# Ham3798/shielded-pool-pinocchio-solana

Hardware: AMD Instinct MI355X
Metric: Groth16 proofs/sec (higher is better)
Workload: dtype u32x8 (254-bit Montgomery integers); 1 GPU; audit_circuit (RLWE, const-PK; scripts/generate_audit.py:246-465), batch of 2048 independent proofs per GPU per step, every row a distinct witness; circuit=audit, n_constraints=29178, n_wires=35432, domain=32768, batch_per_gpu=2048, n_distinct_witnesses=2048, table_bytes=226725433344, parallelism=independent proofs x1, pk_bytes=9850060

## Files before the change

include/spp.h:

```cpp
#ifndef SPP_H
#define SPP_H
#include <stddef.h>
#include <stdint.h>
#ifdef __cplusplus
extern "C" {
#endif

#define SPP_OK 0
#define SPP_ERR_BAD_INPUT (-1)
#define SPP_ERR_NO_DEVICE (-2)
#define SPP_ERR_IO (-3)
#define SPP_ERR_UNSAT (-4)
#define SPP_ERR_HIP (-5)
#define SPP_ERR_NOT_IMPLEMENTED (-6)
#define SPP_ERR_FORMAT (-7)

#define SPP_CIRCUIT_WITHDRAW 1
#define SPP_CIRCUIT_AUDIT 2
#define SPP_CIRCUIT_WITHDRAW_REFSHAPE 3
#define SPP_CIRCUIT_WITHDRAW_DEPTH20 4

#define SPP_PROOF_LEN 388
#define SPP_WITHDRAW_PW_LEN 172
#define SPP_AUDIT_PW_LEN 76
// ... 142 lines not shown
int  spp_pool_submit_audit_batch(spp_pool*, size_t count, const uint8_t* proofs, const uint8_t* pws, int32_t* result);
int  spp_pool_withdraw_batch(spp_pool*, size_t count, const uint8_t* proofs, const uint8_t* pws, const uint8_t* recipients,
                             int32_t* result, uint64_t* amounts);
#define SPP_INSTR_DEPOSIT 0
#define SPP_INSTR_SUBMIT_AUDIT 1
#define SPP_INSTR_WITHDRAW 2
int  spp_pool_settle_log(spp_pool*, size_t count, const uint8_t* kinds,
                         size_t n_deposits, const uint8_t* roots,
                         size_t n_audits, const uint8_t* audit_proofs, const uint8_t* audit_pws,
                         size_t n_withdraws, const uint8_t* withdraw_proofs, const uint8_t* withdraw_pws, const uint8_t* recipients,
                         int32_t* result, uint64_t* amounts);

int spp_ntt_fr(spp_ctx* ctx, uint8_t* data, uint32_t logn, int inverse);
int spp_msm_g1(spp_ctx* ctx, const uint8_t* bases, const uint8_t* scalars, size_t n, int window_bits, uint8_t out[64]);
int spp_msm_g2(spp_ctx* ctx, const uint8_t* bases, const uint8_t* scalars, size_t n, int window_bits, uint8_t out[128]);

int spp_msm_g1_pippenger(spp_ctx* ctx, const uint8_t* bases, const uint8_t* scalars, size_t n, uint8_t out[64]);
int spp_msm_g2_pippenger(spp_ctx* ctx, const uint8_t* bases, const uint8_t* scalars, size_t n, uint8_t out[128]);
int spp_msm_g1_pippenger_bench(spp_ctx* ctx, size_t n, uint64_t seed, const uint8_t scale_be[32], int iters, uint8_t out[64],
                               float* ms_total, float* ms_bucket_kernel);
int spp_msm_g1_pippenger_bench_dist(spp_ctx* ctx, size_t n, uint64_t seed, uint32_t small_permille, const uint8_t scale_be[32], int iters,
                                    uint8_t out[64], float* ms_total, float* ms_bucket_kernel);
int spp_msm_g1_pippenger_bench_shard(spp_ctx* ctx, size_t n_total, size_t first, size_t count, uint64_t seed, uint32_t small_permille,
                                     const uint8_t scale_be[32], int iters, uint8_t out[64], float* ms_total, float* ms_bucket_kernel);

#ifdef __cplusplus
}
#endif
#endif
```

shielded-pool-pinocchio-solana_amd/csrc/f29.hpp:

```cpp
#pragma once
#include "bn254.hpp"

#if defined(__HIPCC__)
#define SPP_HD_COLD __host__ __device__ __attribute__((noinline))
#else
#define SPP_HD_COLD __attribute__((noinline))
#endif

namespace spp {

template <class Pm>
struct F29 {
  uint32_t l[9];
  using Base = Fp<Pm>;
  typedef uint32_t (*ConstFn)(int);
  static constexpr uint32_t M = (1u << 29) - 1u;
  static constexpr uint32_t INV = Pm::INV32 & M;
  static SPP_HD constexpr uint32_t P9(int k) { return Base::P9(k); }

  template <ConstFn C>
  static SPP_HD F29 konst() {
    F29 r;
    SPP_UNROLL for (int i = 0; i < 9; i++) r.l[i] = C(i);
    return r;
// ... 176 lines not shown
  }
  SPP_HD XYZZ<B> to_xyzz() const {
    if (inf) return XYZZ<B>::infinity();
    return {X.to_fp(), Y.to_fp(), ZZ.scaled_to_fp(), ZZZ.scaled_to_fp()};
  }
  static SPP_HD XYZZ29 from_xyzz(const XYZZ<B>& q) {
    XYZZ29 r;
    r.inf = q.is_inf();
    r.X = F::from_fp(q.X);
    r.Y = F::from_fp(q.Y);
    r.ZZ = F::from_fp(q.ZZ) * F::template konst<Pm::K29_IN>();
    r.ZZZ = F::from_fp(q.ZZZ) * F::template konst<Pm::K29_IN>();
    return r;
  }

  SPP_HD void madd(const Affine<B>& e, bool negate) {
    F x2 = F::from_words(e.x.l);
    F y2 = F::from_words(e.y.l);
    if (negate) y2 = F::template neg_lazy<Pm::SUBC_4P_1>(y2);
    if (inf) {
      X = x2 * F::template konst<Pm::K29_IN>();
      Y = y2 * F::template konst<Pm::K29_IN>();
      ZZ = F::template konst<Pm::K29_IN>();
      ZZZ = ZZ;
      inf = false;
      return;
    }
    const F U2 = x2 * ZZ;
    const F Pp = F::template sub_norm<Pm::SUBC_6P_1>(U2, X);
    if (Pp.template is_zero_mod_p<7>()) {
      const F S2 = y2 * ZZZ;
      const F Rr = F::template sub_norm<Pm::SUBC_2P_1>(S2, Y);
      if (Rr.template is_zero_mod_p<3>()) {
        XYZZ<B> t = to_xyzz();
        t.dbl_inplace();
        const XYZZ29 d = from_xyzz(t);
        X = d.X;
        Y = d.Y;
        ZZ = d.ZZ;
        ZZZ = d.ZZZ;
      } else {
        inf = true;
      }
      return;
    }
    const F PP = Pp.sqr();
    const F Q = X * PP;
    const F PPP = Pp * PP;
    ZZ = ZZ * PP;
    const F S2 = y2 * ZZZ;
    const F Rr = F::template sub_norm<Pm::SUBC_2P_1>(S2, Y);
    ZZZ = ZZZ * PPP;
    const F R2 = Rr.sqr();
    X = F::template sub3_norm<Pm::SUBC_4P_3>(R2, PPP, Q);
    const F T = F::template sub_lazy<Pm::SUBC_6P_1>(Q, X);
    const F Yn = F::template neg_lazy<Pm::SUBC_2P_1>(Y);
    Y = F::mul2(Rr, T, Yn, PPP);
  }
};

struct F29x2 {
  using F = F29<FqParams>;
  using Pm = FqParams;
  F c0, c1;

  static SPP_HD F29x2 from_words(const Fq2& a) { return {F::from_words(a.c0.l), F::from_words(a.c1.l)}; }
  template <F::ConstFn CA>
  static SPP_HD F29x2 mul(const F29x2& a, const F29x2& b) {
    const F na1 = F::template neg_lazy<CA>(a.c1);
    return {F::mul2(a.c0, b.c0, na1, b.c1), F::mul2(a.c0, b.c1, a.c1, b.c0)};
  }
  SPP_HD F29x2 mul_real(const F& k) const { return {c0 * k, c1 * k}; }
// ... 44 lines not shown
  SPP_HD XYZZ<Fq2> to_xyzz() const {
    if (inf) return XYZZ<Fq2>::infinity();
    return {X.to_fp(), Y.to_fp(), ZZ.scaled_to_fp(), ZZZ.scaled_to_fp()};
  }
  static SPP_HD XYZZ29G2 from_xyzz(const XYZZ<Fq2>& q) {
    XYZZ29G2 r;
    r.inf = q.is_inf();
    const F k = F::template konst<Pm::K29_IN>();
    r.X = E::from_fp(q.X);
    r.Y = E::from_fp(q.Y);
    r.ZZ = E::from_fp(q.ZZ).mul_real(k);
    r.ZZZ = E::from_fp(q.ZZZ).mul_real(k);
    return r;
  }

  SPP_HD void madd(const Affine<Fq2>& e, bool negate) {
    const E x2 = E::from_words(e.x);
    const E y2 = E::from_words(e.y);
    if (inf) {
      const F k = F::template konst<Pm::K29_IN>();
      X = x2.mul_real(k);
      const E yn = E::template neg_lazy<Pm::SUBC_4P_1>(y2);
      E ys;
      SPP_UNROLL for (int i = 0; i < 9; i++) {
        ys.c0.l[i] = negate ? yn.c0.l[i] : y2.c0.l[i];
        ys.c1.l[i] = negate ? yn.c1.l[i] : y2.c1.l[i];
      }
      Y = ys.mul_real(k);
      SPP_UNROLL for (int i = 0; i < 9; i++) {
        ZZ.c0.l[i] = k.l[i];
        ZZ.c1.l[i] = 0;
      }
      ZZZ = ZZ;
      inf = false;
      return;
    }
    const E U2 = E::template mul<Pm::SUBC_4P_1>(x2, ZZ);
    const E Pp = E::template sub_norm<Pm::SUBC_6P_1>(U2, X);
    E S2 = E::template mul<Pm::SUBC_4P_1>(y2, ZZZ);
    if (negate) S2 = E::template neg_lazy<Pm::SUBC_2P_1>(S2);
    const E Rr = E::template sub_norm<Pm::SUBC_2P_1>(S2, Y);
    if (Pp.template is_zero_mod_p<7>()) {
      if (Rr.template is_zero_mod_p<4>()) {
        XYZZ<Fq2> t = to_xyzz();
        t.dbl_inplace();
        const XYZZ29G2 d = from_xyzz(t);
        X = d.X;
        Y = d.Y;
        ZZ = d.ZZ;
        ZZZ = d.ZZZ;
      } else {
        inf = true;
      }
      return;
    }
    const E PP = Pp.template sqr<Pm::SUBC_8P_1>();
    const E Q = E::template mul<Pm::SUBC_6P_1>(X, PP);
    const E PPP = E::template mul<Pm::SUBC_8P_1>(Pp, PP);
    ZZ = E::template mul<Pm::SUBC_2P_1>(ZZ, PP);
    ZZZ = E::template mul<Pm::SUBC_2P_1>(ZZZ, PPP);
    const E R2 = Rr.template sqr<Pm::SUBC_6P_1>();
    X = E::template sub3_norm<Pm::SUBC_4P_3>(R2, PPP, Q);
    const E T = E::template sub_norm<Pm::SUBC_6P_1>(Q, X);
    const F nR1 = F::template neg_lazy<Pm::SUBC_6P_1>(Rr.c1);
    const F nY0 = F::template neg_lazy<Pm::SUBC_2P_1>(Y.c0);
    const F nY1 = F::template neg_lazy<Pm::SUBC_2P_1>(Y.c1);
    uint64_t c[18];
    F::clear(c);
    F::mac(c, Rr.c0, T.c0);
    F::mac(c, nR1, T.c1);
    F::mac(c, nY0, PPP.c0);
    F::mac(c, Y.c1, PPP.c1);
    const F y0 = F::reduce(c);
    F::clear(c);
    F::mac(c, Rr.c0, T.c1);
    F::mac(c, Rr.c1, T.c0);
    F::mac(c, nY0, PPP.c1);
    F::mac(c, nY1, PPP.c0);
    Y.c0 = y0;
    Y.c1 = F::reduce(c);
  }
};

}
```

shielded-pool-pinocchio-solana_amd/csrc/kernels.hpp:

```cpp
#pragma once
#include <hip/hip_runtime.h>
#include <stdint.h>
#include "bn254.hpp"
#include "msm_plan.hpp"
#include "msm_ragged.hpp"
#include "rlwe_ntt.hpp"

namespace spp {

struct DevSparse {
  const uint32_t* rowptr;
  const uint32_t* wire;
  const uint32_t* coeff;
  const uint32_t* lit;
};
static constexpr uint32_t COEFF_ONE = 0x80000000u;
static constexpr uint32_t COEFF_MINUS_ONE = 0x40000000u;
static constexpr uint32_t COEFF_MASK = 0x3fffffffu;

struct DevCircuit {
  DevSparse A, B, C, H;
  const Fr* coeffs;
  const Fr* aux;
  const uint32_t* program;
// ... 124 lines not shown
void launch_pool_commit(hipStream_t st, const PoolSet& set, uint64_t salt, const uint8_t* keys, uint32_t stride, uint32_t count, const int32_t* result,
                        uint32_t* set_count);
void launch_spmv_check(hipStream_t st, DevCircuit dc, const Fr* W, Fr* abc, uint32_t n, uint32_t P, uint32_t* status, int16_t* small = nullptr);

void launch_ntt(hipStream_t st, Fr* data, uint32_t logn, uint32_t P, const Fr* tw, bool dif, uint32_t nbatch, size_t batch_stride,
                const Fr* post = nullptr);
void launch_scale_rows(hipStream_t st, Fr* data, const Fr* table, uint32_t n, uint32_t P, uint32_t nbatch, size_t batch_stride);
void launch_qap_pointwise(hipStream_t st, Fr* abc, uint32_t n, uint32_t P, Fr zinv);
void launch_qap_product(hipStream_t st, Fr* abc, uint32_t n, uint32_t P);

template <class F>
struct MsmWalk;
template <>
struct MsmWalk<Fq> {
  static constexpr uint32_t waves_per_simd = 2;
  static constexpr bool gather_ahead = false;
};
template <>
struct MsmWalk<Fq2> {
  static constexpr uint32_t waves_per_simd = 1;
  static constexpr bool gather_ahead = true;
};
template <class F>
void launch_build_table(hipStream_t st, const Affine<F>* bases, uint32_t N, uint32_t c, uint32_t Wt, uint32_t row0, uint32_t nrows,
                        Affine<F>* table, XYZZ<F>* tmp, F* tmp_pre, const MsmBlock* blocks = nullptr, uint32_t E = 0);
void launch_msm_digits(hipStream_t st, const uint32_t* rows, const Fr* scalars, int16_t* dig, uint32_t N, uint32_t P, uint32_t c);
template <class F>
void launch_msm_accumulate(hipStream_t st, const Affine<F>* table, const MsmBlock* blocks, const int16_t* dig, XYZZ<F>* partial, uint32_t N, uint32_t P,
                           uint32_t c, const MsmPlan& pl, hipEvent_t ev_start = nullptr, hipEvent_t ev_stop = nullptr);
template <class F>
void launch_msm_reduce(hipStream_t st, XYZZ<F>* partial, XYZZ<F>* out, uint32_t P, const MsmPlan& pl, uint32_t c, bool empty);
static constexpr uint32_t MSM_FOLD_SETS = 8;
static constexpr uint32_t MSM_FOLD_RADIX = 8;
template <class F>
struct MsmFoldSets {
  XYZZ<F>* partial[MSM_FOLD_SETS];
  XYZZ<F>* out[MSM_FOLD_SETS];
  uint32_t Sg[MSM_FOLD_SETS], R[MSM_FOLD_SETS], c[MSM_FOLD_SETS];
  uint32_t cur[MSM_FOLD_SETS], half[MSM_FOLD_SETS];
};
template <class F>
void launch_msm_reduce_multi(hipStream_t st, MsmFoldSets<F> fs, uint32_t nsets, uint32_t P);

void launch_g1_eval_basis(hipStream_t st, const G1Affine* pts, uint32_t n_pts, uint32_t logn, const Fr* scale, const Fr* tw_inv, G1XYZZ* work,
// ... 34 lines not shown
```

shielded-pool-pinocchio-solana_amd/csrc/kernels_msm.hip:

```cpp
#include "msm_table.hpp"

namespace spp {

template void launch_build_table<Fq>(hipStream_t, const Affine<Fq>*, uint32_t, uint32_t, uint32_t, uint32_t, uint32_t, Affine<Fq>*,
                                     XYZZ<Fq>*, Fq*, const MsmBlock*, uint32_t);
template void launch_msm_accumulate<Fq>(hipStream_t, const Affine<Fq>*, const MsmBlock*, const int16_t*, XYZZ<Fq>*, uint32_t, uint32_t, uint32_t,
                                        const MsmPlan&, hipEvent_t, hipEvent_t);
template void launch_msm_reduce_multi<Fq>(hipStream_t, MsmFoldSets<Fq>, uint32_t, uint32_t);
template void launch_msm_reduce<Fq>(hipStream_t, XYZZ<Fq>*, XYZZ<Fq>*, uint32_t, const MsmPlan&, uint32_t, bool);
template void launch_fixed_base_mul<Fq>(hipStream_t, const Affine<Fq>*, uint32_t, const Fr*, uint32_t, Affine<Fq>*);

__global__ void __launch_bounds__(256) k_msm_digits(const uint32_t* __restrict__ rows, const Fr* __restrict__ scalars,
                                                    int16_t* __restrict__ dig, uint32_t N, uint32_t P, uint32_t Pp, uint32_t c, uint32_t W) {
  const uint64_t g = (uint64_t)blockIdx.x * blockDim.x + threadIdx.x;
  const uint32_t p = (uint32_t)(g % Pp), i = (uint32_t)(g / Pp);
  if (i >= N || p >= P) return;
  const Fr s = scalars[(size_t)rows[i] * P + p];
  uint32_t l[8];
  s.to_canonical(l);
  const bool neg = canonical_gt_half<FrParams>(l);
  if (neg) {
    uint32_t t[8];
    canonical_negate<FrParams>(l, t);
    SPP_UNROLL for (int k = 0; k < 8; k++) l[k] = t[k];
// ... 96 lines not shown
```

shielded-pool-pinocchio-solana_amd/csrc/kernels_msm_g2.hip:

```cpp
#include "msm_table.hpp"

namespace spp {

template void launch_build_table<Fq2>(hipStream_t, const Affine<Fq2>*, uint32_t, uint32_t, uint32_t, uint32_t, uint32_t, Affine<Fq2>*,
                                     XYZZ<Fq2>*, Fq2*, const MsmBlock*, uint32_t);
template void launch_msm_accumulate<Fq2>(hipStream_t, const Affine<Fq2>*, const MsmBlock*, const int16_t*, XYZZ<Fq2>*, uint32_t, uint32_t, uint32_t,
                                        const MsmPlan&, hipEvent_t, hipEvent_t);
template void launch_msm_reduce_multi<Fq2>(hipStream_t, MsmFoldSets<Fq2>, uint32_t, uint32_t);
template void launch_msm_reduce<Fq2>(hipStream_t, XYZZ<Fq2>*, XYZZ<Fq2>*, uint32_t, const MsmPlan&, uint32_t, bool);
template void launch_fixed_base_mul<Fq2>(hipStream_t, const Affine<Fq2>*, uint32_t, const Fr*, uint32_t, Affine<Fq2>*);

}
```

shielded-pool-pinocchio-solana_amd/csrc/msm_table.hpp:

```cpp
#pragma once
#include <hip/hip_ext.h>
#include "kernels.hpp"
#include <algorithm>
#include "f29.hpp"

namespace spp {

static constexpr unsigned MSM_FOLD_COOP_MAX_BATCH = 8;
static constexpr unsigned MSM_WALK_BLOCK = 64;

template <class F>
__global__ void __launch_bounds__(64) k_build_table(const Affine<F>* __restrict__ bases, uint32_t N, uint32_t E, uint32_t Wn,
                                                    uint32_t step_bits, uint32_t row0, uint32_t nrows, Affine<F>* __restrict__ table,
                                                    XYZZ<F>* __restrict__ tmp, F* __restrict__ tmp_pre, const MsmBlock* __restrict__ blocks) {
  const uint32_t rl = blockIdx.x * blockDim.x + threadIdx.x;
  if (rl >= nrows) return;
  const uint32_t row = row0 + rl;
  const size_t off = blocks ? (size_t)blocks[row >> 6].off : (size_t)(row >> 6) * E;
  Affine<F>* out = table + off * 64 + (row & 63);
  XYZZ<F>* t = tmp + rl;
  F* pre = tmp_pre + rl;
  if (row >= N * Wn) {
    for (uint32_t d = 0; d < E; d++) out[(size_t)d * 64] = Affine<F>::infinity();
    return;
// ... 71 lines not shown
__device__ __forceinline__ bool words_all_zero(const Fq& v) {
  uint32_t o = 0;
  SPP_UNROLL for (int i = 0; i < 8; i++) o |= v.l[i];
  return o == 0;
}
template <class F>
struct MsmAcc;
template <>
struct MsmAcc<Fq> {
  XYZZ29<FqParams> a;
  __device__ __forceinline__ void init() { a = XYZZ29<FqParams>::infinity(); }
  __device__ __forceinline__ void madd(const Affine<Fq>& e, bool sgn) {
    if (words_all_zero(e.x) && words_all_zero(e.y)) return;
    a.madd(e, sgn);
  }
  __device__ __forceinline__ XYZZ<Fq> result() const { return a.to_xyzz(); }
};

template <>
struct MsmAcc<Fq2> {
  XYZZ29G2 a;
  __device__ __forceinline__ void init() { a = XYZZ29G2::infinity(); }
  __device__ __forceinline__ void madd(const Affine<Fq2>& e, bool sgn) {
    if (words_all_zero(e.x.c0) && words_all_zero(e.x.c1) && words_all_zero(e.y.c0) && words_all_zero(e.y.c1)) return;
    a.madd(e, sgn);
  }
  __device__ __forceinline__ XYZZ<Fq2> result() const { return a.to_xyzz(); }
};


template <class F>
__global__ void __launch_bounds__(MSM_WALK_BLOCK, MsmWalk<F>::waves_per_simd) k_msm_flat(const Affine<F>* __restrict__ table, const MsmBlock* __restrict__ blocks,
                                                  const int16_t* __restrict__ dig, XYZZ<F>* __restrict__ partial, uint32_t N, uint32_t P,
                                                  uint32_t Pp, uint32_t R, uint32_t Sg) {
  const uint32_t g = blockIdx.x * blockDim.x + threadIdx.x;
  const uint32_t p = g % Pp, t = g / Pp;
  if (t >= R * Sg || p >= P) return;
  const uint32_t rho = t / Sg, sl = t % Sg;
  const int16_t* __restrict__ dg = dig + ((size_t)rho * N) * Pp + p;
  MsmAcc<F> acc;
  acc.init();
  if constexpr (MsmWalk<F>::gather_ahead) {
    int d_next = 0;
    Affine<F> e_next;
    for (uint32_t i0 = sl;; i0 += 4 * Sg) {
      const bool last = i0 >= N;
      uint64_t pack = 0;
      if (!last) {
        SPP_UNROLL for (uint32_t k = 0; k < 4; k++) {
          const uint32_t i = i0 + k * Sg;
          const uint32_t d = i < N ? (uint32_t)(uint16_t)dg[(size_t)i * Pp] : 0u;
          pack |= (uint64_t)d << (16 * k);
        }
      }
#pragma unroll 1
      for (uint32_t k = 0; k < 4; k++) {
        int d = (int)(int16_t)(uint16_t)(pack >> (16 * k));
        const bool flush = last && k == 0;
        const uint32_t i = i0 + k * Sg;
        const uint32_t mag = (uint32_t)(d < 0 ? -d : d);
        MsmBlock blk{};
        if (d != 0) blk = blocks[i >> 6];
        if (mag > blk.E) d = 0;
        if (d != 0 || flush) {
          Affine<F> e;
          if (d != 0) e = table[((size_t)blk.off + (mag - 1)) * 64 + (i & 63)];
          if (d_next != 0) acc.madd(e_next, d_next < 0);
          d_next = d;
          if (d != 0) e_next = e;
        }
      }
      if (last) break;
    }
  } else {
    for (uint32_t i0 = sl; i0 < N; i0 += 4 * Sg) {
      uint64_t pack = 0;
      SPP_UNROLL for (uint32_t k = 0; k < 4; k++) {
        const uint32_t i = i0 + k * Sg;
        const uint32_t d = i < N ? (uint32_t)(uint16_t)dg[(size_t)i * Pp] : 0u;
        pack |= (uint64_t)d << (16 * k);
      }
      if (pack == 0) continue;
#pragma unroll 1
      for (uint32_t k = 0; k < 4; k++) {
        const int d = (int)(int16_t)(uint16_t)(pack >> (16 * k));
        if (d != 0) {
          const uint32_t i = i0 + k * Sg;
          const uint32_t mag = (uint32_t)(d < 0 ? -d : d);
          const MsmBlock blk = blocks[i >> 6];
          if (mag <= blk.E) acc.madd(table[((size_t)blk.off + (mag - 1)) * 64 + (i & 63)], d < 0);
        }
      }
    }
  }
  partial[(size_t)t * P + p] = acc.result();
}

template <class F>
__global__ void __launch_bounds__(256) k_msm_rows(const Affine<F>* __restrict__ table, const int16_t* __restrict__ dig,
                                                  XYZZ<F>* __restrict__ partial, uint32_t N, uint32_t P, uint32_t Pp, uint32_t c,
                                                  uint32_t Wt, uint32_t R, uint32_t W, uint32_t Sg, uint32_t Q, uint32_t Wq) {
  const uint32_t g = blockIdx.x * blockDim.x + threadIdx.x;
  const uint32_t p = g % Pp, t = g / Pp;
  if (t >= R * Sg || p >= P) return;
  const uint32_t rho = t / Sg, sl = t % Sg;
  const uint32_t E = 1u << (c - 1);
  const size_t plane = (size_t)N * Pp;
  MsmAcc<F> acc;
  acc.init();
  const uint32_t items = N * Q;
// ... 10 lines not shown
      const uint32_t j = rho + R * m;
      if (j >= W) break;
      const int d = dg[(size_t)j * plane];
      if (d != 0) {
        const uint32_t row = i * Wt + m;
        const uint32_t mag = (uint32_t)(d < 0 ? -d : d);
        acc.madd(table[((size_t)(row >> 6) * E + (mag - 1)) * 64 + (row & 63)], d < 0);
      }
    }
  }
  partial[(size_t)t * P + p] = acc.result();
}

template <class F>
void launch_msm_accumulate(hipStream_t st, const Affine<F>* table, const MsmBlock* blocks, const int16_t* dig, XYZZ<F>* partial, uint32_t N, uint32_t P,
                           uint32_t c, const MsmPlan& pl, hipEvent_t ev_start, hipEvent_t ev_stop) {
  if (N == 0 || P == 0) {
    if (ev_start) hipEventRecord(ev_start, st);
    if (ev_stop) hipEventRecord(ev_stop, st);
    return;
  }
  const uint64_t lanes = (uint64_t)pl.R * pl.Sg * pl.Pp;
  if (pl.Wt == 1)
    hipExtLaunchKernelGGL(k_msm_flat<F>, dim3((uint32_t)((lanes + MSM_WALK_BLOCK - 1) / MSM_WALK_BLOCK)), dim3(MSM_WALK_BLOCK), 0, st, ev_start, ev_stop, 0, table, blocks, dig, partial, N, P, pl.Pp, pl.R, pl.Sg);
  else
    hipExtLaunchKernelGGL(k_msm_rows<F>, dim3((uint32_t)((lanes + 255) / 256)), dim3(256), 0, st, ev_start, ev_stop, 0, table, dig, partial, N, P, pl.Pp, c,
                          pl.Wt, pl.R, pl.W, pl.Sg, pl.Q, pl.Wq);
}

template <class T>
__device__ __forceinline__ T msm_shfl_xor(const T& v, int mask) {
  static_assert(sizeof(T) % 4 == 0, "word-sized");
  T r;
  const uint32_t* s = reinterpret_cast<const uint32_t*>(&v);
  uint32_t* d = reinterpret_cast<uint32_t*>(&r);
  SPP_UNROLL for (uint32_t i = 0; i < sizeof(T) / 4; i++) d[i] = (uint32_t)__shfl_xor((int)s[i], mask, 64);
  return r;
}
template <class F>
__global__ void __launch_bounds__(64) k_msm_fold_multi(MsmFoldSets<F> fs, uint32_t P, uint32_t coop) {
// ... 158 lines not shown
```

shielded-pool-pinocchio-solana_amd/csrc/spp_load.cpp:

```cpp
#include "spp_circuit.hpp"

static std::vector<PendingTable<Fq>>& pending(spp_circuit* c, Fq*) { return c->pending1; }
static std::vector<PendingTable<Fq2>>& pending(spp_circuit* c, Fq2*) { return c->pending2; }

static int upload_sparse(spp_circuit* c, const Circuit& circ, const Sparse& m, DevSparse* out) {
  std::vector<uint32_t> wire(m.terms.size()), coeff(m.terms.size()), lit(m.terms.size(), 0);
  Fr one = Fr::one(), mone = Fr::one().neg();
  std::vector<uint32_t> small(circ.coeffs.size(), 0);
  for (size_t ci = 0; ci < circ.coeffs.size(); ci++) {
    uint32_t v[8], nv[8];
    circ.coeffs[ci].to_canonical(v);
    bool hi0 = true;
    for (int k = 1; k < 8; k++) hi0 = hi0 && v[k] == 0;
    if (hi0 && v[0] != 0 && v[0] < (1u << 28)) { small[ci] = v[0]; continue; }
    circ.coeffs[ci].neg().to_canonical(nv);
    hi0 = true;
    for (int k = 1; k < 8; k++) hi0 = hi0 && nv[k] == 0;
    if (hi0 && nv[0] != 0 && nv[0] < (1u << 28)) small[ci] = nv[0] | 0x80000000u;
  }
  for (size_t i = 0; i < m.terms.size(); i++) {
    wire[i] = m.terms[i].wire;
    uint32_t ci = m.terms[i].coeff;
    uint32_t flag = 0;
    if (circ.coeffs[ci] == one) flag = COEFF_ONE;
// ... 798 lines not shown
  std::vector<uint32_t> rows(n);
  for (size_t i = 0; i < n; i++) {
    pts[i] = point_from_raw<F>(bases + PT_BYTES * i);
    sc[i] = Fr::from_bytes_be(scalars + 32 * i);
    rows[i] = (uint32_t)i;
  }
  spp_circuit tmpc;
  tmpc.ctx = ctx;
  tmpc.c_bits = cb;
  Affine<F>* table = nullptr;
  int e = build_table_chunked<F>(&tmpc, pts, cb, Wn, &table);
  Fr* d_sc = nullptr;
  uint32_t* d_rows = nullptr;
  XYZZ<F> *partial = nullptr, *d_out = nullptr;
  DevBuf dig;
  const MsmPlan pl = msm_plan((uint32_t)n, 1, cb, Wn, MsmWalk<F>::waves_per_simd, read_switches().msm);
  if (!e) e = own_upload(&tmpc, &d_sc, sc);
  if (!e) e = own_upload(&tmpc, &d_rows, rows);
  if (!e && hipMalloc((void**)&partial, sizeof(XYZZ<F>) * std::max<size_t>(pl.partial_elems(1), 1)) != hipSuccess) e = fail(SPP_ERR_HIP, "hipMalloc");
  if (!e && hipMalloc((void**)&d_out, sizeof(XYZZ<F>)) != hipSuccess) e = fail(SPP_ERR_HIP, "hipMalloc");
  if (!e && dig.alloc(sizeof(int16_t) * std::max<size_t>(msm_digit_elems((uint32_t)n, 1, cb), 1)) != hipSuccess) e = fail(SPP_ERR_HIP, "hipMalloc");
  XYZZ<F> res = XYZZ<F>::infinity();
  if (!e) {
    launch_msm_digits(st, d_rows, d_sc, dig.as<int16_t>(), (uint32_t)n, 1, cb);
    launch_msm_accumulate<F>(st, table, nullptr, dig.as<int16_t>(), partial, (uint32_t)n, 1, cb, pl);
    launch_msm_reduce<F>(st, partial, d_out, 1, pl, cb, n == 0);
    if (hipStreamSynchronize(st) != hipSuccess || hipGetLastError() != hipSuccess) e = fail(SPP_ERR_HIP, "msm kernels failed");
    else if (hipMemcpy(&res, d_out, sizeof res, hipMemcpyDeviceToHost) != hipSuccess) e = fail(SPP_ERR_HIP, "copy back failed");
  }
  for (void* p : tmpc.owned) hipFree(p);
  if (partial) hipFree(partial);
  if (d_out) hipFree(d_out);
  if (e) return e;
  point_to_raw(res.to_affine(), out);
  return SPP_OK;
}
extern "C" int spp_msm_g1(spp_ctx* ctx, const uint8_t* bases, const uint8_t* scalars, size_t n, int window_bits, uint8_t out[64]) {
  return msm_fixed_unit<Fq, 64>(ctx, bases, scalars, n, window_bits, out);
}
extern "C" int spp_msm_g2(spp_ctx* ctx, const uint8_t* bases, const uint8_t* scalars, size_t n, int window_bits, uint8_t out[128]) {
  return msm_fixed_unit<Fq2, 128>(ctx, bases, scalars, n, window_bits, out);
}
```

shielded-pool-pinocchio-solana_amd/csrc/spp_prove.cpp:

```cpp
#include "spp_circuit.hpp"

template <class T>
static int ws_alloc(Workspace& w, T** p, size_t count) {
  HIP_TRY(hipMalloc((void**)p, sizeof(T) * std::max<size_t>(count, 1)));
  w.owned.push_back((void*)*p);
  return 0;
}
template <class F>
static int ws_set(const spp_circuit* c, Workspace& w, const MsmSet<F>* s, MsmBuf<F>* b, size_t P) {
  b->partial_cap = msm_partial_cap(s->N, P, s->c, s->Wt, MsmWalk<F>::waves_per_simd, c->sw.msm);
  int e;
  if ((e = ws_alloc(w, &b->partial, b->partial_cap))) return e;
  return ws_alloc(w, &b->out, P);
}
static int ensure_workspace(spp_circuit* c, Workspace& w, size_t P) {
  if (P <= w.cap) return 0;
  HIP_TRY(hipStreamSynchronize(w.st));
  free_workspace(w);
  int e;
  if ((e = ws_alloc(w, &w.W, (size_t)c->n_rows * P)) || (e = ws_alloc(w, &w.abc, (size_t)3 * c->n * P)) ||
      (e = ws_alloc(w, &w.scratch, (size_t)c->max_batch_div * P)) || (e = ws_alloc(w, &w.commit_affine, P)) ||
      (e = ws_alloc(w, &w.d_inputs, c->in_stride * P)) || (e = ws_alloc(w, &w.d_rs, 64 * P)) ||
      (e = ws_alloc(w, &w.d_proofs, (size_t)SPP_PROOF_LEN * P)) || (e = ws_alloc(w, &w.d_pws, c->pw_stride * P)) ||
      (e = ws_alloc(w, &w.d_status, P)) || (e = ws_alloc(w, &w.counters, 256 * P)))
    return e;
// ... 14 lines not shown
    w.dig2_cap = msm_digit_elems(c->B2.N, (uint32_t)P, c->B2.c);
    if ((e = ws_alloc(w, &w.dig1, w.dig1_cap)) || (e = ws_alloc(w, &w.dig2, w.dig2_cap))) return e;
    if (c->dc.sm_nrows && (e = ws_alloc(w, &w.small, (size_t)c->dc.sm_nslots * P))) return e;
  }
  w.cap = P;
  return 0;
}

static int16_t* ws_dig(Workspace& w, Fq*) { return w.dig1; }
static int16_t* ws_dig(Workspace& w, Fq2*) { return w.dig2; }
template <class F>
static void run_msm(spp_circuit* c, Workspace& w, const MsmSet<F>& s, MsmBuf<F>& b, uint32_t P, bool timed, hipStream_t st_override = nullptr,
                    std::pair<hipEvent_t, hipEvent_t>* ev_override = nullptr, bool fold = true, const Fr* scal_override = nullptr) {
  hipStream_t st = st_override ? st_override : w.st;
  const Fr* scal = scal_override ? scal_override : s.from_h ? w.abc : w.W;
  MsmPlan pl = msm_plan(s.N, P, s.c, s.Wt, MsmWalk<F>::waves_per_simd, c->sw.msm);
  pl.fit(P, b.partial_cap);
  b.plan = pl;
  std::pair<hipEvent_t, hipEvent_t>* ev = nullptr;
  if (timed && w.msm_ev_used < w.msm_ev.size()) ev = &w.msm_ev[w.msm_ev_used++];
  if (ev_override) ev = ev_override;
  int16_t* dig = ws_dig(w, (F*)nullptr);
  launch_msm_digits(st, s.rows, scal, dig, s.N, P, s.c);
  launch_msm_accumulate<F>(st, s.table, s.blocks, dig, b.partial, s.N, P, s.c, pl, ev ? ev->first : nullptr, ev ? ev->second : nullptr);
  if (fold) launch_msm_reduce<F>(st, b.partial, b.out, P, pl, s.c, s.N == 0);
}

static int prove_on_device(spp_circuit* c, Workspace& w, uint32_t P, const uint8_t* d_inputs, const uint8_t* d_rs, uint8_t* d_proofs,
                           uint8_t* d_pws, uint32_t* d_status) {
  hipStream_t st = w.st;
  const Circuit& circ = c->circ;
// ... 495 lines not shown
```

shielded-pool-pinocchio-solana_amd/spp/lib.py:

```python
import ctypes
import os

_HERE = os.path.dirname(os.path.abspath(__file__))
LIB_PATH = os.path.join(os.path.dirname(_HERE), "libspp.so")
_LIB = None

SPP_OK = 0
SPP_ERR_UNSAT = -4
SPP_CIRCUIT_WITHDRAW = 1
SPP_CIRCUIT_AUDIT = 2
SPP_CIRCUIT_WITHDRAW_DEPTH20 = 4
SPP_CIRCUIT_WITHDRAW_REFSHAPE = 3
PROOF_LEN = 388
NOTE_LEN = 160
DEPOSIT_LEN = 96
AUDIT_PW_LEN = 76
SPP_AUDIT_BAD_PROOF = 1
SPP_AUDIT_BAD_CIPHERTEXT = 2
SPP_AUDIT_BAD_IDENTITY = 4
WITHDRAW_PW_LEN = 172
SPP_POOL_STATE_LEN = 1072
SPP_POOL_NULLIFIERS = 0
SPP_POOL_AUDIT_RECORDS = 1
SPP_POOL_OK = 0
# ... 97 lines not shown
    L.spp_pool_state.argtypes = [vp, vp]
    L.spp_pool_counts.argtypes = [vp, vp]
    L.spp_pool_import_keys.argtypes = [vp, i32, sz, cp]
    L.spp_pool_contains.argtypes = [vp, i32, sz, cp, vp]
    L.spp_pool_submit_audit_batch.argtypes = [vp, sz, cp, cp, vp]
    L.spp_pool_withdraw_batch.argtypes = [vp, sz, cp, cp, cp, vp, vp]
    L.spp_pool_settle_log.argtypes = [vp, sz, cp, sz, cp, sz, cp, cp, sz, cp, cp, cp, vp, vp]
    L.spp_withdraw_rows_from_tree.argtypes = [vp, sz, cp, vp]
    L.spp_prove_withdraw_notes_device.argtypes = [vp, vp, sz, vp, vp, vp, vp, vp]
    L.spp_prove_withdraw_notes.argtypes = [vp, vp, sz, cp, cp, vp, vp, vp]
    L.spp_shamir_reconstruct.argtypes = [vp, u32, vp, cp, sz, vp, vp]
    L.spp_rlwe_decrypt_batch.argtypes = [vp, vp, sz, vp, vp, vp]
    L.spp_ntt_fr.argtypes = [vp, vp, u32, i32]
    L.spp_msm_g1.argtypes = [vp, cp, cp, sz, i32, vp]
    L.spp_msm_g2.argtypes = [vp, cp, cp, sz, i32, vp]
    L.spp_msm_g1_pippenger.argtypes = [vp, cp, cp, sz, vp]
    L.spp_msm_g2_pippenger.argtypes = [vp, cp, cp, sz, vp]
    L.spp_msm_g1_pippenger_bench.argtypes = [vp, sz, ctypes.c_uint64, cp, i32, vp, ctypes.POINTER(ctypes.c_float), ctypes.POINTER(ctypes.c_float)]
    L.spp_msm_g1_pippenger_bench_dist.argtypes = [vp, sz, ctypes.c_uint64, ctypes.c_uint32, cp, i32, vp, ctypes.POINTER(ctypes.c_float),
                                                  ctypes.POINTER(ctypes.c_float)]
    L.spp_msm_g1_pippenger_bench_shard.argtypes = [vp, sz, sz, sz, ctypes.c_uint64, ctypes.c_uint32, cp, i32, vp, ctypes.POINTER(ctypes.c_float),
                                                   ctypes.POINTER(ctypes.c_float)]
    _LIB = L
    return L


def last_error():
    return load_library().spp_last_error().decode()


# ... 4 lines not shown
```

shielded-pool-pinocchio-solana_amd/spp/prover.py:

```python
import ctypes
import numpy as np
from .lib import load_library, check, SppError, PROOF_LEN, SPP_ERR_UNSAT, AUDIT_PW_LEN


def build_circuit(circuit_id, out_path, aux=None):
    L = load_library()
    n = ctypes.c_uint32(0)
    auxbuf = None
    if aux is not None:
        auxbuf = (ctypes.c_uint32 * len(aux))(*[int(v) for v in aux])
    check(L.spp_circuit_build(int(circuit_id), auxbuf, out_path.encode(), ctypes.byref(n)))
    return n.value


def verify(vk_bytes, proof_bytes, pw_bytes):
    L = load_library()
    ok = ctypes.c_int(0)
    check(L.spp_verify(vk_bytes, len(vk_bytes), proof_bytes, len(proof_bytes), pw_bytes, len(pw_bytes), ctypes.byref(ok)))
    return bool(ok.value)


def pairing_check_host(pairs):
    L = load_library()
    ok = ctypes.c_int(0)
# ... 39 lines not shown
        check(self.L.spp_ntt_fr(self.h, ctypes.cast(buf, ctypes.c_void_p), logn, 1 if inverse else 0))
        return [int.from_bytes(buf.raw[32 * i:32 * i + 32], "big") for i in range(n)]

    def msm_g1(self, bases_bytes, scalars, window_bits=8):
        n = len(scalars)
        out = ctypes.create_string_buffer(64)
        sc = b"".join(int(s).to_bytes(32, "big") for s in scalars)
        check(self.L.spp_msm_g1(self.h, bases_bytes, sc, n, int(window_bits), ctypes.cast(out, ctypes.c_void_p)))
        return out.raw

    def msm_g2(self, bases_bytes, scalars, window_bits=8):
        out = ctypes.create_string_buffer(128)
        sc = b"".join(int(s).to_bytes(32, "big") for s in scalars)
        check(self.L.spp_msm_g2(self.h, bases_bytes, sc, len(scalars), int(window_bits), ctypes.cast(out, ctypes.c_void_p)))
        return out.raw

    def msm_g1_pippenger(self, bases_bytes, scalars):
        out = ctypes.create_string_buffer(64)
        sc = b"".join(int(s).to_bytes(32, "big") for s in scalars)
        check(self.L.spp_msm_g1_pippenger(self.h, bases_bytes, sc, len(scalars), ctypes.cast(out, ctypes.c_void_p)))
        return out.raw

    def msm_g2_pippenger(self, bases_bytes, scalars):
        out = ctypes.create_string_buffer(128)
        sc = b"".join(int(s).to_bytes(32, "big") for s in scalars)
        check(self.L.spp_msm_g2_pippenger(self.h, bases_bytes, sc, len(scalars), ctypes.cast(out, ctypes.c_void_p)))
        return out.raw

    def pairing_check(self, pairs):
        ok = ctypes.c_int(0)
# ... 203 lines not shown
```

Measured before the change: 6735 proofs/s.

## Split flat MSM walk into distinct-add fast path with redo kernel fallback

Measured after the change: 7048 proofs/s, median of 6. 1.05x the previous value.

```diff
diff --git a/include/spp.h b/include/spp.h
--- a/include/spp.h
+++ b/include/spp.h
@@ -180,6 +180,8 @@
 int spp_ntt_fr(spp_ctx* ctx, uint8_t* data, uint32_t logn, int inverse);
 int spp_msm_g1(spp_ctx* ctx, const uint8_t* bases, const uint8_t* scalars, size_t n, int window_bits, uint8_t out[64]);
 int spp_msm_g2(spp_ctx* ctx, const uint8_t* bases, const uint8_t* scalars, size_t n, int window_bits, uint8_t out[128]);
+int spp_msm_flat_unit(spp_ctx* ctx, int group, const uint8_t* bases, size_t n, const uint8_t* scalars, size_t P, int window_bits, uint8_t* out,
+                      uint32_t* redo_lanes);
 
 int spp_msm_g1_pippenger(spp_ctx* ctx, const uint8_t* bases, const uint8_t* scalars, size_t n, uint8_t out[64]);
 int spp_msm_g2_pippenger(spp_ctx* ctx, const uint8_t* bases, const uint8_t* scalars, size_t n, uint8_t out[128]);
diff --git a/shielded-pool-pinocchio-solana_amd/csrc/f29.hpp b/shielded-pool-pinocchio-solana_amd/csrc/f29.hpp
--- a/shielded-pool-pinocchio-solana_amd/csrc/f29.hpp
+++ b/shielded-pool-pinocchio-solana_amd/csrc/f29.hpp
@@ -214,7 +214,10 @@
     return r;
   }
 
-  SPP_HD void madd(const Affine<B>& e, bool negate) {
+  SPP_HD void madd(const Affine<B>& e, bool negate) { madd_any<false>(e, negate); }
+  SPP_HD bool madd_distinct(const Affine<B>& e, bool negate) { return madd_any<true>(e, negate); }
+  template <bool DISTINCT>
+  SPP_HD bool madd_any(const Affine<B>& e, bool negate) {
     F x2 = F::from_words(e.x.l);
     F y2 = F::from_words(e.y.l);
     if (negate) y2 = F::template neg_lazy<Pm::SUBC_4P_1>(y2);
@@ -224,11 +227,12 @@
       ZZ = F::template konst<Pm::K29_IN>();
       ZZZ = ZZ;
       inf = false;
-      return;
+      return true;
     }
     const F U2 = x2 * ZZ;
     const F Pp = F::template sub_norm<Pm::SUBC_6P_1>(U2, X);
     if (Pp.template is_zero_mod_p<7>()) {
+      if constexpr (DISTINCT) return false;
       const F S2 = y2 * ZZZ;
       const F Rr = F::template sub_norm<Pm::SUBC_2P_1>(S2, Y);
       if (Rr.template is_zero_mod_p<3>()) {
@@ -242,7 +246,7 @@
       } else {
         inf = true;
       }
-      return;
+      return true;
     }
     const F PP = Pp.sqr();
     const F Q = X * PP;
@@ -256,6 +260,7 @@
     const F T = F::template sub_lazy<Pm::SUBC_6P_1>(Q, X);
     const F Yn = F::template neg_lazy<Pm::SUBC_2P_1>(Y);
     Y = F::mul2(Rr, T, Yn, PPP);
+    return true;
   }
 };
 
@@ -330,7 +335,10 @@
     return r;
   }
 
-  SPP_HD void madd(const Affine<Fq2>& e, bool negate) {
+  SPP_HD void madd(const Affine<Fq2>& e, bool negate) { madd_any<false>(e, negate); }
+  SPP_HD bool madd_distinct(const Affine<Fq2>& e, bool negate) { return madd_any<true>(e, negate); }
+  template <bool DISTINCT>
+  SPP_HD bool madd_any(const Affine<Fq2>& e, bool negate) {
     const E x2 = E::from_words(e.x);
     const E y2 = E::from_words(e.y);
     if (inf) {
@@ -349,7 +357,7 @@
       }
       ZZZ = ZZ;
       inf = false;
-      return;
+      return true;
     }
     const E U2 = E::template mul<Pm::SUBC_4P_1>(x2, ZZ);
     const E Pp = E::template sub_norm<Pm::SUBC_6P_1>(U2, X);
@@ -357,6 +365,7 @@
     if (negate) S2 = E::template neg_lazy<Pm::SUBC_2P_1>(S2);
     const E Rr = E::template sub_norm<Pm::SUBC_2P_1>(S2, Y);
     if (Pp.template is_zero_mod_p<7>()) {
+      if constexpr (DISTINCT) return false;
       if (Rr.template is_zero_mod_p<4>()) {
         XYZZ<Fq2> t = to_xyzz();
         t.dbl_inplace();
@@ -368,7 +377,7 @@
       } else {
         inf = true;
       }
-      return;
+      return true;
     }
     const E PP = Pp.template sqr<Pm::SUBC_8P_1>();
     const E Q = E::template mul<Pm::SUBC_6P_1>(X, PP);
@@ -395,6 +404,7 @@
     F::mac(c, nY1, PPP.c0);
     Y.c0 = y0;
     Y.c1 = F::reduce(c);
+    return true;
   }
 };
 
diff --git a/shielded-pool-pinocchio-solana_amd/csrc/kernels.hpp b/shielded-pool-pinocchio-solana_amd/csrc/kernels.hpp
--- a/shielded-pool-pinocchio-solana_amd/csrc/kernels.hpp
+++ b/shielded-pool-pinocchio-solana_amd/csrc/kernels.hpp
@@ -162,12 +162,16 @@
 template <>
 struct MsmWalk<Fq> {
   static constexpr uint32_t waves_per_simd = 2;
+  static constexpr uint32_t rows_waves_per_simd = 2;
   static constexpr bool gather_ahead = false;
+  static constexpr uint32_t occ(uint32_t Wt) { return Wt == 1 ? waves_per_simd : rows_waves_per_simd; }
 };
 template <>
 struct MsmWalk<Fq2> {
-  static constexpr uint32_t waves_per_simd = 1;
-  static constexpr bool gather_ahead = true;
+  static constexpr uint32_t waves_per_simd = 2;
+  static constexpr uint32_t rows_waves_per_simd = 1;
+  static constexpr bool gather_ahead = false;
+  static constexpr uint32_t occ(uint32_t Wt) { return Wt == 1 ? waves_per_simd : rows_waves_per_simd; }
 };
 template <class F>
 void launch_build_table(hipStream_t st, const Affine<F>* bases, uint32_t N, uint32_t c, uint32_t Wt, uint32_t row0, uint32_t nrows,
@@ -175,7 +179,7 @@
 void launch_msm_digits(hipStream_t st, const uint32_t* rows, const Fr* scalars, int16_t* dig, uint32_t N, uint32_t P, uint32_t c);
 template <class F>
 void launch_msm_accumulate(hipStream_t st, const Affine<F>* table, const MsmBlock* blocks, const int16_t* dig, XYZZ<F>* partial, uint32_t N, uint32_t P,
-                           uint32_t c, const MsmPlan& pl, hipEvent_t ev_start = nullptr, hipEvent_t ev_stop = nullptr);
+                           uint32_t c, const MsmPlan& pl, hipEvent_t ev_start = nullptr, hipEvent_t ev_stop = nullptr, uint32_t* redo_count = nullptr);
 template <class F>
 void launch_msm_reduce(hipStream_t st, XYZZ<F>* partial, XYZZ<F>* out, uint32_t P, const MsmPlan& pl, uint32_t c, bool empty);
 static constexpr uint32_t MSM_FOLD_SETS = 8;
diff --git a/shielded-pool-pinocchio-solana_amd/csrc/kernels_msm.hip b/shielded-pool-pinocchio-solana_amd/csrc/kernels_msm.hip
--- a/shielded-pool-pinocchio-solana_amd/csrc/kernels_msm.hip
+++ b/shielded-pool-pinocchio-solana_amd/csrc/kernels_msm.hip
@@ -5,7 +5,7 @@
 template void launch_build_table<Fq>(hipStream_t, const Affine<Fq>*, uint32_t, uint32_t, uint32_t, uint32_t, uint32_t, Affine<Fq>*,
                                      XYZZ<Fq>*, Fq*, const MsmBlock*, uint32_t);
 template void launch_msm_accumulate<Fq>(hipStream_t, const Affine<Fq>*, const MsmBlock*, const int16_t*, XYZZ<Fq>*, uint32_t, uint32_t, uint32_t,
-                                        const MsmPlan&, hipEvent_t, hipEvent_t);
+                                        const MsmPlan&, hipEvent_t, hipEvent_t, uint32_t*);
 template void launch_msm_reduce_multi<Fq>(hipStream_t, MsmFoldSets<Fq>, uint32_t, uint32_t);
 template void launch_msm_reduce<Fq>(hipStream_t, XYZZ<Fq>*, XYZZ<Fq>*, uint32_t, const MsmPlan&, uint32_t, bool);
 template void launch_fixed_base_mul<Fq>(hipStream_t, const Affine<Fq>*, uint32_t, const Fr*, uint32_t, Affine<Fq>*);
diff --git a/shielded-pool-pinocchio-solana_amd/csrc/kernels_msm_g2.hip b/shielded-pool-pinocchio-solana_amd/csrc/kernels_msm_g2.hip
--- a/shielded-pool-pinocchio-solana_amd/csrc/kernels_msm_g2.hip
+++ b/shielded-pool-pinocchio-solana_amd/csrc/kernels_msm_g2.hip
@@ -5,7 +5,7 @@
 template void launch_build_table<Fq2>(hipStream_t, const Affine<Fq2>*, uint32_t, uint32_t, uint32_t, uint32_t, uint32_t, Affine<Fq2>*,
                                      XYZZ<Fq2>*, Fq2*, const MsmBlock*, uint32_t);
 template void launch_msm_accumulate<Fq2>(hipStream_t, const Affine<Fq2>*, const MsmBlock*, const int16_t*, XYZZ<Fq2>*, uint32_t, uint32_t, uint32_t,
-                                        const MsmPlan&, hipEvent_t, hipEvent_t);
+                                        const MsmPlan&, hipEvent_t, hipEvent_t, uint32_t*);
 template void launch_msm_reduce_multi<Fq2>(hipStream_t, MsmFoldSets<Fq2>, uint32_t, uint32_t);
 template void launch_msm_reduce<Fq2>(hipStream_t, XYZZ<Fq2>*, XYZZ<Fq2>*, uint32_t, const MsmPlan&, uint32_t, bool);
 template void launch_fixed_base_mul<Fq2>(hipStream_t, const Affine<Fq2>*, uint32_t, const Fr*, uint32_t, Affine<Fq2>*);
diff --git a/shielded-pool-pinocchio-solana_amd/csrc/msm_table.hpp b/shielded-pool-pinocchio-solana_amd/csrc/msm_table.hpp
--- a/shielded-pool-pinocchio-solana_amd/csrc/msm_table.hpp
+++ b/shielded-pool-pinocchio-solana_amd/csrc/msm_table.hpp
@@ -109,6 +109,10 @@
     if (words_all_zero(e.x) && words_all_zero(e.y)) return;
     a.madd(e, sgn);
   }
+  __device__ __forceinline__ bool madd_distinct(const Affine<Fq>& e, bool sgn) {
+    if (words_all_zero(e.x) && words_all_zero(e.y)) return true;
+    return a.madd_distinct(e, sgn);
+  }
   __device__ __forceinline__ XYZZ<Fq> result() const { return a.to_xyzz(); }
 };
 
@@ -120,22 +124,32 @@
     if (words_all_zero(e.x.c0) && words_all_zero(e.x.c1) && words_all_zero(e.y.c0) && words_all_zero(e.y.c1)) return;
     a.madd(e, sgn);
   }
+  __device__ __forceinline__ bool madd_distinct(const Affine<Fq2>& e, bool sgn) {
+    if (words_all_zero(e.x.c0) && words_all_zero(e.x.c1) && words_all_zero(e.y.c0) && words_all_zero(e.y.c1)) return true;
+    return a.madd_distinct(e, sgn);
+  }
   __device__ __forceinline__ XYZZ<Fq2> result() const { return a.to_xyzz(); }
 };
 
 
 template <class F>
-__global__ void __launch_bounds__(MSM_WALK_BLOCK, MsmWalk<F>::waves_per_simd) k_msm_flat(const Affine<F>* __restrict__ table, const MsmBlock* __restrict__ blocks,
-                                                  const int16_t* __restrict__ dig, XYZZ<F>* __restrict__ partial, uint32_t N, uint32_t P,
-                                                  uint32_t Pp, uint32_t R, uint32_t Sg) {
-  const uint32_t g = blockIdx.x * blockDim.x + threadIdx.x;
-  const uint32_t p = g % Pp, t = g / Pp;
-  if (t >= R * Sg || p >= P) return;
-  const uint32_t rho = t / Sg, sl = t % Sg;
-  const int16_t* __restrict__ dg = dig + ((size_t)rho * N) * Pp + p;
-  MsmAcc<F> acc;
-  acc.init();
-  if constexpr (MsmWalk<F>::gather_ahead) {
+__device__ __forceinline__ void msm_store_redo_marker(XYZZ<F>* out) {
+  static_assert(sizeof(XYZZ<F>) % 16 == 0, "stored as 16-byte words");
+  uint4* w = reinterpret_cast<uint4*>(out);
+  SPP_UNROLL for (uint32_t i = 0; i < sizeof(XYZZ<F>) / 16; i++) w[i] = make_uint4(0, 0, 0, 0);
+}
+template <class F>
+__device__ __forceinline__ bool msm_is_redo_marker(const XYZZ<F>* v) {
+  const uint32_t* x = reinterpret_cast<const uint32_t*>(&v->X);
+  const uint32_t* zz = reinterpret_cast<const uint32_t*>(&v->ZZ);
+  uint32_t o = 0;
+  SPP_UNROLL for (uint32_t i = 0; i < sizeof(F) / 4; i++) o |= x[i] | zz[i];
+  return o == 0;
+}
+template <class F, bool FAST>
+__device__ __forceinline__ bool msm_flat_walk(MsmAcc<F>& acc, const Affine<F>* __restrict__ table, const MsmBlock* __restrict__ blocks,
+                                              const int16_t* __restrict__ dg, uint32_t N, uint32_t Pp, uint32_t sl, uint32_t Sg) {
+  if constexpr (FAST && MsmWalk<F>::gather_ahead) {
     int d_next = 0;
     Affine<F> e_next;
     for (uint32_t i0 = sl;; i0 += 4 * Sg) {
@@ -160,7 +174,7 @@
         if (d != 0 || flush) {
           Affine<F> e;
           if (d != 0) e = table[((size_t)blk.off + (mag - 1)) * 64 + (i & 63)];
-          if (d_next != 0) acc.madd(e_next, d_next < 0);
+          if (d_next != 0 && !acc.madd_distinct(e_next, d_next < 0)) return false;
           d_next = d;
           if (d != 0) e_next = e;
         }
@@ -183,12 +197,48 @@
           const uint32_t i = i0 + k * Sg;
           const uint32_t mag = (uint32_t)(d < 0 ? -d : d);
           const MsmBlock blk = blocks[i >> 6];
-          if (mag <= blk.E) acc.madd(table[((size_t)blk.off + (mag - 1)) * 64 + (i & 63)], d < 0);
+          if (mag <= blk.E) {
+            const Affine<F> e = table[((size_t)blk.off + (mag - 1)) * 64 + (i & 63)];
+            if constexpr (FAST) {
+              if (!acc.madd_distinct(e, d < 0)) return false;
+            } else {
+              acc.madd(e, d < 0);
+            }
+          }
         }
       }
     }
   }
-  partial[(size_t)t * P + p] = acc.result();
+  return true;
+}
+template <class F>
+__global__ void __launch_bounds__(MSM_WALK_BLOCK, MsmWalk<F>::waves_per_simd) k_msm_flat(const Affine<F>* __restrict__ table, const MsmBlock* __restrict__ blocks,
+                                                  const int16_t* __restrict__ dig, XYZZ<F>* __restrict__ partial, uint32_t N, uint32_t P,
+                                                  uint32_t Pp, uint32_t R, uint32_t Sg) {
+  const uint32_t g = blockIdx.x * blockDim.x + threadIdx.x;
+  const uint32_t p = g % Pp, t = g / Pp;
+  if (t >= R * Sg || p >= P) return;
+  const uint32_t rho = t / Sg, sl = t % Sg;
+  MsmAcc<F> acc;
+  acc.init();
+  if (msm_flat_walk<F, true>(acc, table, blocks, dig + ((size_t)rho * N) * Pp + p, N, Pp, sl, Sg)) partial[(size_t)t * P + p] = acc.result();
+  else msm_store_redo_marker(partial + (size_t)t * P + p);
+}
+template <class F>
+__global__ void __launch_bounds__(MSM_WALK_BLOCK, MsmWalk<F>::waves_per_simd) k_msm_flat_redo(const Affine<F>* __restrict__ table, const MsmBlock* __restrict__ blocks,
+                                                  const int16_t* __restrict__ dig, XYZZ<F>* __restrict__ partial, uint32_t N, uint32_t P,
+                                                  uint32_t Pp, uint32_t R, uint32_t Sg, uint32_t* __restrict__ redo_count) {
+  const uint32_t g = blockIdx.x * blockDim.x + threadIdx.x;
+  const uint32_t p = g % Pp, t = g / Pp;
+  if (t >= R * Sg || p >= P) return;
+  XYZZ<F>* out = partial + (size_t)t * P + p;
+  if (!msm_is_redo_marker(out)) return;
+  if (redo_count) atomicAdd(redo_count, 1u);
+  const uint32_t rho = t / Sg, sl = t % Sg;
+  MsmAcc<F> acc;
+  acc.init();
+  msm_flat_walk<F, false>(acc, table, blocks, dig + ((size_t)rho * N) * Pp + p, N, Pp, sl, Sg);
+  *out = acc.result();
 }
 
 template <class F>
@@ -229,16 +279,18 @@
 
 template <class F>
 void launch_msm_accumulate(hipStream_t st, const Affine<F>* table, const MsmBlock* blocks, const int16_t* dig, XYZZ<F>* partial, uint32_t N, uint32_t P,
-                           uint32_t c, const MsmPlan& pl, hipEvent_t ev_start, hipEvent_t ev_stop) {
+                           uint32_t c, const MsmPlan& pl, hipEvent_t ev_start, hipEvent_t ev_stop, uint32_t* redo_count) {
   if (N == 0 || P == 0) {
     if (ev_start) hipEventRecord(ev_start, st);
     if (ev_stop) hipEventRecord(ev_stop, st);
     return;
   }
   const uint64_t lanes = (uint64_t)pl.R * pl.Sg * pl.Pp;
-  if (pl.Wt == 1)
-    hipExtLaunchKernelGGL(k_msm_flat<F>, dim3((uint32_t)((lanes + MSM_WALK_BLOCK - 1) / MSM_WALK_BLOCK)), dim3(MSM_WALK_BLOCK), 0, st, ev_start, ev_stop, 0, table, blocks, dig, partial, N, P, pl.Pp, pl.R, pl.Sg);
-  else
+  if (pl.Wt == 1) {
+    const dim3 grid((uint32_t)((lanes + MSM_WALK_BLOCK - 1) / MSM_WALK_BLOCK));
+    hipExtLaunchKernelGGL(k_msm_flat<F>, grid, dim3(MSM_WALK_BLOCK), 0, st, ev_start, ev_stop, 0, table, blocks, dig, partial, N, P, pl.Pp, pl.R, pl.Sg);
+    hipLaunchKernelGGL(k_msm_flat_redo<F>, grid, dim3(MSM_WALK_BLOCK), 0, st, table, blocks, dig, partial, N, P, pl.Pp, pl.R, pl.Sg, redo_count);
+  } else
     hipExtLaunchKernelGGL(k_msm_rows<F>, dim3((uint32_t)((lanes + 255) / 256)), dim3(256), 0, st, ev_start, ev_stop, 0, table, dig, partial, N, P, pl.Pp, c,
                           pl.Wt, pl.R, pl.W, pl.Sg, pl.Q, pl.Wq);
 }
diff --git a/shielded-pool-pinocchio-solana_amd/csrc/spp_load.cpp b/shielded-pool-pinocchio-solana_amd/csrc/spp_load.cpp
--- a/shielded-pool-pinocchio-solana_amd/csrc/spp_load.cpp
+++ b/shielded-pool-pinocchio-solana_amd/csrc/spp_load.cpp
@@ -836,7 +836,7 @@
   uint32_t* d_rows = nullptr;
   XYZZ<F> *partial = nullptr, *d_out = nullptr;
   DevBuf dig;
-  const MsmPlan pl = msm_plan((uint32_t)n, 1, cb, Wn, MsmWalk<F>::waves_per_simd, read_switches().msm);
+  const MsmPlan pl = msm_plan((uint32_t)n, 1, cb, Wn, MsmWalk<F>::occ(Wn), read_switches().msm);
   if (!e) e = own_upload(&tmpc, &d_sc, sc);
   if (!e) e = own_upload(&tmpc, &d_rows, rows);
   if (!e && hipMalloc((void**)&partial, sizeof(XYZZ<F>) * std::max<size_t>(pl.partial_elems(1), 1)) != hipSuccess) e = fail(SPP_ERR_HIP, "hipMalloc");
@@ -863,3 +863,66 @@
 extern "C" int spp_msm_g2(spp_ctx* ctx, const uint8_t* bases, const uint8_t* scalars, size_t n, int window_bits, uint8_t out[128]) {
   return msm_fixed_unit<Fq2, 128>(ctx, bases, scalars, n, window_bits, out);
 }
+
+template <class F, size_t PT_BYTES>
+static int msm_flat_unit(spp_ctx* ctx, const uint8_t* bases, size_t n, const uint8_t* scalars, size_t P, int window_bits, uint8_t* out,
+                         uint32_t* redo_lanes) {
+  if (!ctx || !out || !bases || !scalars || n == 0 || P == 0) return fail(SPP_ERR_BAD_INPUT, "NULL or empty argument");
+  if (window_bits == 0) window_bits = 8;
+  if (window_bits < 4 || window_bits > 16) return fail(SPP_ERR_BAD_INPUT, "window_bits outside [4,16]");
+  if (n > (1u << 20) || P > (1u << 16)) return fail(SPP_ERR_BAD_INPUT, "too many bases or rows");
+  std::lock_guard<std::mutex> lk(ctx->mu);
+  HIP_TRY(hipSetDevice(ctx->device));
+  hipStream_t st = ctx->stream;
+  const uint32_t cb = (uint32_t)window_bits, N = (uint32_t)n, Pn = (uint32_t)P, E = 1u << (cb - 1);
+  if ((uint64_t)msm_table_elems(N, cb, 1) * PT_BYTES > ((uint64_t)64 << 30)) return fail(SPP_ERR_BAD_INPUT, "table would exceed 64 GiB; use a smaller window");
+  std::vector<Affine<F>> pts(n);
+  std::vector<Fr> sc(n * P);
+  std::vector<uint32_t> rows(n);
+  for (size_t i = 0; i < n; i++) {
+    pts[i] = point_from_raw<F>(bases + PT_BYTES * i);
+    rows[i] = (uint32_t)i;
+    for (size_t p = 0; p < P; p++) sc[i * P + p] = Fr::from_bytes_be(scalars + 32 * (p * n + i));
+  }
+  std::vector<MsmBlock> blocks(msm_table_rows(n, 1) / 64);
+  for (size_t b = 0; b < blocks.size(); b++) blocks[b] = {(uint64_t)b * E, E, 0};
+  spp_circuit tmpc;
+  tmpc.ctx = ctx;
+  tmpc.c_bits = cb;
+  Affine<F>* table = nullptr;
+  int e = build_table_chunked<F>(&tmpc, pts, cb, 1, &table);
+  Fr* d_sc = nullptr;
+  uint32_t* d_rows = nullptr;
+  MsmBlock* d_blocks = nullptr;
+  const MsmPlan pl = msm_plan(N, Pn, cb, 1, MsmWalk<F>::occ(1), read_switches().msm);
+  DevBuf partial, d_out, dig, count;
+  if (!e) e = own_upload(&tmpc, &d_sc, sc);
+  if (!e) e = own_upload(&tmpc, &d_rows, rows);
+  if (!e) e = own_upload(&tmpc, &d_blocks, blocks);
+  if (!e && (partial.alloc(sizeof(XYZZ<F>) * pl.partial_elems(Pn)) != hipSuccess || d_out.alloc(sizeof(XYZZ<F>) * P) != hipSuccess ||
+             dig.alloc(sizeof(int16_t) * msm_digit_elems(N, Pn, cb)) != hipSuccess || count.alloc(sizeof(uint32_t)) != hipSuccess))
+    e = fail(SPP_ERR_HIP, "hipMalloc");
+  std::vector<XYZZ<F>> res(P);
+  uint32_t redone = 0;
+  if (!e) {
+    hipMemsetAsync(count.p, 0, sizeof(uint32_t), st);
+    launch_msm_digits(st, d_rows, d_sc, dig.as<int16_t>(), N, Pn, cb);
+    launch_msm_accumulate<F>(st, table, d_blocks, dig.as<int16_t>(), partial.as<XYZZ<F>>(), N, Pn, cb, pl, nullptr, nullptr, count.as<uint32_t>());
+    launch_msm_reduce<F>(st, partial.as<XYZZ<F>>(), d_out.as<XYZZ<F>>(), Pn, pl, cb, false);
+    if (hipStreamSynchronize(st) != hipSuccess || hipGetLastError() != hipSuccess) e = fail(SPP_ERR_HIP, "msm kernels failed");
+    else if (hipMemcpy(res.data(), d_out.p, sizeof(XYZZ<F>) * P, hipMemcpyDeviceToHost) != hipSuccess ||
+             hipMemcpy(&redone, count.p, sizeof redone, hipMemcpyDeviceToHost) != hipSuccess)
+      e = fail(SPP_ERR_HIP, "copy back failed");
+  }
+  for (void* p : tmpc.owned) hipFree(p);
+  if (e) return e;
+  for (size_t p = 0; p < P; p++) point_to_raw(res[p].to_affine(), out + PT_BYTES * p);
+  if (redo_lanes) *redo_lanes = redone;
+  return SPP_OK;
+}
+extern "C" int spp_msm_flat_unit(spp_ctx* ctx, int group, const uint8_t* bases, size_t n, const uint8_t* scalars, size_t P, int window_bits,
+                                 uint8_t* out, uint32_t* redo_lanes) {
+  if (group == 1) return msm_flat_unit<Fq, 64>(ctx, bases, n, scalars, P, window_bits, out, redo_lanes);
+  if (group == 2) return msm_flat_unit<Fq2, 128>(ctx, bases, n, scalars, P, window_bits, out, redo_lanes);
+  return fail(SPP_ERR_BAD_INPUT, "group is 1 or 2");
+}
diff --git a/shielded-pool-pinocchio-solana_amd/csrc/spp_prove.cpp b/shielded-pool-pinocchio-solana_amd/csrc/spp_prove.cpp
--- a/shielded-pool-pinocchio-solana_amd/csrc/spp_prove.cpp
+++ b/shielded-pool-pinocchio-solana_amd/csrc/spp_prove.cpp
@@ -8,7 +8,7 @@
 }
 template <class F>
 static int ws_set(const spp_circuit* c, Workspace& w, const MsmSet<F>* s, MsmBuf<F>* b, size_t P) {
-  b->partial_cap = msm_partial_cap(s->N, P, s->c, s->Wt, MsmWalk<F>::waves_per_simd, c->sw.msm);
+  b->partial_cap = msm_partial_cap(s->N, P, s->c, s->Wt, MsmWalk<F>::occ(s->Wt), c->sw.msm);
   int e;
   if ((e = ws_alloc(w, &b->partial, b->partial_cap))) return e;
   return ws_alloc(w, &b->out, P);
@@ -53,7 +53,7 @@
                     std::pair<hipEvent_t, hipEvent_t>* ev_override = nullptr, bool fold = true, const Fr* scal_override = nullptr) {
   hipStream_t st = st_override ? st_override : w.st;
   const Fr* scal = scal_override ? scal_override : s.from_h ? w.abc : w.W;
-  MsmPlan pl = msm_plan(s.N, P, s.c, s.Wt, MsmWalk<F>::waves_per_simd, c->sw.msm);
+  MsmPlan pl = msm_plan(s.N, P, s.c, s.Wt, MsmWalk<F>::occ(s.Wt), c->sw.msm);
   pl.fit(P, b.partial_cap);
   b.plan = pl;
   std::pair<hipEvent_t, hipEvent_t>* ev = nullptr;
diff --git a/shielded-pool-pinocchio-solana_amd/spp/lib.py b/shielded-pool-pinocchio-solana_amd/spp/lib.py
--- a/shielded-pool-pinocchio-solana_amd/spp/lib.py
+++ b/shielded-pool-pinocchio-solana_amd/spp/lib.py
@@ -135,6 +135,7 @@
     L.spp_ntt_fr.argtypes = [vp, vp, u32, i32]
     L.spp_msm_g1.argtypes = [vp, cp, cp, sz, i32, vp]
     L.spp_msm_g2.argtypes = [vp, cp, cp, sz, i32, vp]
+    L.spp_msm_flat_unit.argtypes = [vp, i32, cp, sz, cp, sz, i32, vp, ctypes.POINTER(ctypes.c_uint32)]
     L.spp_msm_g1_pippenger.argtypes = [vp, cp, cp, sz, vp]
     L.spp_msm_g2_pippenger.argtypes = [vp, cp, cp, sz, vp]
     L.spp_msm_g1_pippenger_bench.argtypes = [vp, sz, ctypes.c_uint64, cp, i32, vp, ctypes.POINTER(ctypes.c_float), ctypes.POINTER(ctypes.c_float)]
diff --git a/shielded-pool-pinocchio-solana_amd/spp/prover.py b/shielded-pool-pinocchio-solana_amd/spp/prover.py
--- a/shielded-pool-pinocchio-solana_amd/spp/prover.py
+++ b/shielded-pool-pinocchio-solana_amd/spp/prover.py
@@ -77,6 +77,17 @@
         sc = b"".join(int(s).to_bytes(32, "big") for s in scalars)
         check(self.L.spp_msm_g2(self.h, bases_bytes, sc, len(scalars), int(window_bits), ctypes.cast(out, ctypes.c_void_p)))
         return out.raw
+
+    def msm_flat(self, group, bases_bytes, scalar_rows, window_bits=8):
+        size = 64 if group == 1 else 128
+        n = len(scalar_rows[0])
+        assert all(len(r) == n for r in scalar_rows) and len(bases_bytes) == size * n
+        out = ctypes.create_string_buffer(size * len(scalar_rows))
+        sc = b"".join(int(s).to_bytes(32, "big") for r in scalar_rows for s in r)
+        redo = ctypes.c_uint32(0)
+        check(self.L.spp_msm_flat_unit(self.h, int(group), bases_bytes, n, sc, len(scalar_rows), int(window_bits),
+                                       ctypes.cast(out, ctypes.c_void_p), ctypes.byref(redo)))
+        return [out.raw[size * p:size * (p + 1)] for p in range(len(scalar_rows))], redo.value
 
     def msm_g1_pippenger(self, bases_bytes, scalars):
         out = ctypes.create_string_buffer(64)
```
